# tech-srl/code2vec

Hardware: NVIDIA H100
Metric: path-contexts/sec (train step, batch 1024x200) (higher is better)
Workload: dtype tf32 operands / fp32 accumulate+storage

## Files before the change

### code2vec_b200/csrc/engine.cu

```cuda
#include <cuda_runtime.h>
#include <math.h>
#include <stdio.h>
#include <stdlib.h>
#include <string.h>

#include <string>
#include <utility>
#include <vector>

#include "../../include/c2v_b200.h"
#include "common.cuh"
#include "kernels.cuh"
#include "sgemm.cuh"
#include "umma_gemm.cuh"

using namespace c2v;

namespace {

thread_local std::string g_create_error = "";

constexpr size_t kAlign = 256;
inline size_t align_up(size_t x, size_t a = kAlign) { return (x + a - 1) / a * a; }

// ... 875 lines not shown
    C2V_CUDA(e, cudaEventRecord(e->ev_fork, st));
    C2V_CUDA(e, cudaStreamWaitEvent(e->side, e->ev_fork, 0));
    {
      PhaseTimer pt(e, PH_DX_SCATTER, e->side);
      BucketPlan bp;
      if (e->inbox.world > 1 && plan_buckets(e, &bp, true)) {
        if (e->sorted_src != cs.src || e->sorted_rows != cs.rows) {
          if ((rc = sort_entries(e, e->side, cs, bp))) return rc;
        }
        e->sorted_src = nullptr;
        const int32_t* starts = wsp<int32_t>(e, e->ws.bkt_starts);
        C2V_LAUNCH(e, (inbox_counts_kernel<<<1, 32, 0, e->side>>>(e->inbox, bp, starts)));
        C2V_LAUNCH(e, (scatter_inbox_kernel<<<(3 * N + 7) / 8, 256, 0, e->side>>>(cs, dp, mask, wsp<int32_t>(e, e->ws.perm), starts, bp, dXg,
                                                                              e->inbox, e->grad_scale)));
      } else if (plan_buckets(e, &bp)) {
        if ((rc = sort_entries(e, e->side, cs, bp))) return rc;
        C2V_LAUNCH(e, (scatter_sorted_kernel<<<(3 * N + 7) / 8, 256, 0, e->side>>>(cs, dp, mask, wsp<int32_t>(e, e->ws.perm), dXg, e->gr_tok,
                                                                               e->gr_path, e->grad_scale)));
      } else if (e->deterministic) {
        if ((rc = det_scatter(e, e->side, cs, mask, dp, dXg, false))) return rc;
      } else {
        C2V_LAUNCH(e, (scatter_dx_kernel<<<(N + 7) / 8, 256, 0, e->side>>>(cs, dp, mask, dXg, e->gr_tok, e->gr_path, e->grad_scale)));
      }
    }
    if ((rc = early_catchup(e, e->side))) return rc;
    C2V_CUDA(e, cudaEventRecord(e->ev_join, e->side));
    if ((rc = run_pending_dy(e, st))) return rc;
    {
      PhaseTimer pt(e, PH_DW, st);
      umma::Operand opA{Xg, (size_t)K3, true, x3 ? wsp<float>(e, e->ws.Xg_lo) : nullptr};
      umma::Operand opB{H, (size_t)D, true, H_lo};
      const int ks = umma::effective_splits(N, kSplitDw);
      umma::EpiStore ep{part, (size_t)D, (size_t)K3 * D};
      C2V_LAUNCH(e, C2V_CUDA(e, (umma::launch(st, K3, D, N, kSplitDw, opA, opB, ep, e->num_sms))));
      rc = launch_colsum(e, st, part, (size_t)K3 * D, ks, K3 * D, e->grad.W);
      if (rc) return rc;
    }
    C2V_CUDA(e, cudaStreamWaitEvent(st, e->ev_join, 0));
    if (e->dy_in_flight) {
      C2V_CUDA(e, cudaStreamWaitEvent(st, e->ev_join2, 0));
      e->dy_in_flight = false;
    }
    e->emb_grads_clean = false;
    return C2V_OK;
  }
  {
    PhaseTimer pt(e, PH_DW, st);
    simt::GatherColsX al{cs, dp};
    simt::ColsX bl{H, (size_t)D};
    const int ks = simt::effective_ksplit(N, kSplitDw);
    simt::StoreC ep{part, (size_t)D, (size_t)K3 * D};
    C2V_LAUNCH(e, C2V_CUDA(e, simt::launch(st, K3, D, N, kSplitDw, al, bl, ep)));
    rc = launch_colsum(e, st, part, (size_t)K3 * D, ks, K3 * D, e->grad.W);
    if (rc) return rc;
  }
  {
    if (e->lazy) {
      if (e->lazy_grads_pending)
        return fail(e, C2V_ERR_STATE, "lazy_adam: every train step must be followed by c2v_adam_step before the next one");
      e->lazy_grads_pending = true;
    } else if (!e->emb_grads_clean && e->table_world == 1) {
      C2V_CUDA(e, cudaMemsetAsync(e->grad.tok, 0, (size_t)e->dims.token_vocab * d * 4, st));
      C2V_CUDA(e, cudaMemsetAsync(e->grad.path, 0, (size_t)e->dims.path_vocab * d * 4, st));
    }
    PhaseTimer pt(e, PH_DX_SCATTER, st);
    simt::RowsK al{H, (size_t)D};
    simt::RowsK bl{e->theta.W, (size_t)D};
// ... 40 lines not shown
  }
  simt::RowsK al{S, e->ws.ldS};
  simt::ColsX bl{e->theta.tgt, (size_t)D};
  const int ks = simt::effective_ksplit(Y, kSplitDv);
  simt::StoreC ep{part, (size_t)D, (size_t)B * D};
  C2V_LAUNCH(e, C2V_CUDA(e, simt::launch(st, B, D, Y, kSplitDv, al, bl, ep)));
  return launch_colsum(e, st, part, (size_t)B * D, ks, B * D, dv);
}

int run_dy(c2v_engine* e, cudaStream_t st, const float* v, int B, const SlabDesc& slab) {
  const int D = e->dims.code_dim, Y = e->dims.target_vocab;
  float* S = wsp<float>(e, e->ws.S);
  {
    PhaseTimer pt(e, PH_DY, st);
    if (is_3x(e) && !aligned16(v))
      return fail(e, C2V_ERR_INVALID, "3xTF32: the code vectors must be 16-byte aligned");
    if (is_tc(e) && aligned16(v)) {
      const size_t ldB = align_up((size_t)B, 4);
      int rcs;
      if (is_3x(e)) {
        PhaseTimer pts(e, PH_SPLIT, st);
        rcs = transpose_operand(e, st, v, B, D, ldB, e->ws.vT, true, e->ws.vT_lo);
      } else {
        rcs = transpose_operand(e, st, v, B, D, ldB, e->ws.vT, false);
      }
      if (rcs) return rcs;
      umma::Operand opA{S, e->ws.ldS, true, is_3x(e) ? wsp<float>(e, e->ws.S_lo) : nullptr};
      umma::Operand opB{wsp<float>(e, e->ws.vT), ldB, false, is_3x(e) ? wsp<float>(e, e->ws.vT_lo) : nullptr};
      auto go = [&](auto ep) -> int {
        if (slab.loaders)
          C2V_LAUNCH(e, C2V_CUDA(e, (umma::launch_cfg<true, false, decltype(ep), umma::AXSoftmaxGrad<false>>(
                                        st, Y, D, B, 1, opA, opB, ep, e->num_sms, umma::AXSoftmaxGrad<false>{slab.sg}))));
        else
          C2V_LAUNCH(e, C2V_CUDA(e, (umma::launch_cfg<true, false, decltype(ep)>(st, Y, D, B, 1, opA, opB, ep, e->num_sms))));
        return C2V_OK;
      };
      int rc;
      if (e->tgt_armed && e->has_adam) {
        const double lr_t = (double)e->tgt_lr * sqrt(1.0 - pow((double)e->tgt_b2, (double)e->tgt_t)) /
                            (1.0 - pow((double)e->tgt_b1, (double)e->tgt_t));
        if ((rc = go(umma::EpiAdam{e->theta.tgt, e->am.tgt, e->av.tgt, (size_t)D, (float)lr_t, e->tgt_b1, e->tgt_b2, e->tgt_eps,
                                   1.f - e->tgt_b1, 1.f - e->tgt_b2, e->adam_epi_prefetch})))
          return rc;
        e->tgt_armed = false;
        e->tgt_fused_t = e->tgt_t;
        e->tgt_t_valid = false;
      } else if ((rc = go(umma::EpiStore{e->grad.tgt, (size_t)D, 0}))) {
        return rc;
      }
    } else {
      simt::ColsX al{S, e->ws.ldS};
      simt::ColsX bl{v, (size_t)D};
      simt::StoreC ep{e->grad.tgt, (size_t)D, 0};
      C2V_LAUNCH(e, C2V_CUDA(e, simt::launch(st, Y, D, B, 1, al, bl, ep)));
    }
  }
  if (e->ev_tgt_ready) C2V_CUDA(e, cudaEventRecord(e->ev_tgt_ready, st));
  return C2V_OK;
}

int target_grad_gemms(c2v_engine* e, cudaStream_t st, const float* v, int B, float* dv, const SlabDesc& slab) {
  int rc = run_dv(e, st, B, dv, slab);
  if (rc) return rc;
  if (e->dy_late == 2 && is_tc(e)) {
    C2V_CUDA(e, cudaEventRecord(e->ev_fork2, st));
    C2V_CUDA(e, cudaStreamWaitEvent(e->side2, e->ev_fork2, 0));
    if ((rc = run_dy(e, e->side2, v, B, slab))) return rc;
// ... 972 lines not shown
  C2V_CUDA(e, cudaMemcpyAsync(pth, h_path, nb, cudaMemcpyHostToDevice, st));
  C2V_CUDA(e, cudaMemcpyAsync(tgt, h_tgt, nb, cudaMemcpyHostToDevice, st));
  C2V_CUDA(e, cudaMemcpyAsync(mask, h_mask, nb, cudaMemcpyHostToDevice, st));
  const Dropout dp = make_dropout(e->dims, 1.0f, 0, 0, nullptr);
  if ((rc = forward_impl(e, st, src, pth, tgt, mask, B, dp, code, attn))) return rc;
  if ((rc = topk_impl(e, st, code, B, tki, tkv, normalize))) return rc;
  const int Y = e->dims.target_vocab;
  const int k = e->dims.top_k < Y ? e->dims.top_k : Y;
  C2V_CUDA(e, cudaMemcpyAsync(h_topk_idx, tki, (size_t)B * k * 4, cudaMemcpyDeviceToHost, st));
  C2V_CUDA(e, cudaMemcpyAsync(h_topk_val, tkv, (size_t)B * k * 4, cudaMemcpyDeviceToHost, st));
  if (h_code_vec) C2V_CUDA(e, cudaMemcpyAsync(h_code_vec, code, (size_t)B * e->dims.code_dim * 4, cudaMemcpyDeviceToHost, st));
  if (h_attn) C2V_CUDA(e, cudaMemcpyAsync(h_attn, attn, nb, cudaMemcpyDeviceToHost, st));
  C2V_CUDA(e, cudaStreamSynchronize(st));
  return C2V_OK;
}

int c2v_selftest_gemm(c2v_engine* e, int32_t a_mn, int32_t b_mn, int32_t bn, int32_t M, int32_t N, int32_t K,
                      int32_t splits, const float* A, size_t lda, const float* Bm, size_t ldb, float* C, size_t ldc,
                      void* stream) {
  return c2v_selftest_gemm3(e, a_mn, b_mn, bn, M, N, K, splits, A, nullptr, lda, Bm, nullptr, ldb, C, ldc, stream);
}

int c2v_selftest_gemm3(c2v_engine* e, int32_t a_mn, int32_t b_mn, int32_t bn, int32_t M, int32_t N, int32_t K,
                       int32_t splits, const float* A, const float* A_lo, size_t lda, const float* Bm, const float* B_lo,
                       size_t ldb, float* C, size_t ldc, void* stream) {
  if (!e || !A || !Bm || !C) return C2V_ERR_INVALID;
  if ((A_lo != nullptr) != (B_lo != nullptr)) return fail(e, C2V_ERR_INVALID, "3xTF32 needs the low parts of both operands");
  C2V_CUDA(e, cudaSetDevice(e->device));
  cudaStream_t st = (cudaStream_t)stream;
  umma::Operand opA{A, lda, a_mn != 0, A_lo};
  umma::Operand opB{Bm, ldb, b_mn != 0, B_lo};
  if (!umma::operand_ok(opA) || !umma::operand_ok(opB)) return fail(e, C2V_ERR_INVALID, "operand not TMA-compatible");
  umma::EpiStore ep{C, ldc, (size_t)M * ldc};
  if (bn != 192 && bn != 256) return fail(e, C2V_ERR_INVALID, "bn must be 192 or 256");
  C2V_LAUNCH(e, C2V_CUDA(e, (umma::launch(st, M, N, K, splits, opA, opB, ep, e->num_sms))));
  return umma::effective_splits(K, splits);
}

int c2v_selftest_split(c2v_engine* e, const float* x, float* hi, float* lo, size_t count, void* stream) {
  if (!e || !x || !hi || !lo) return C2V_ERR_INVALID;
  if (count % 4 || ((uintptr_t)x | (uintptr_t)hi | (uintptr_t)lo) % 16) return fail(e, C2V_ERR_INVALID, "count % 4 and 16-byte alignment");
  C2V_CUDA(e, cudaSetDevice(e->device));
  size_t blocks = (count / 4 + 255) / 256;
  if (blocks > (size_t)e->num_sms * 16) blocks = (size_t)e->num_sms * 16;
  if (blocks < 1) blocks = 1;
  C2V_LAUNCH(e, (split_tf32_kernel<<<(unsigned)blocks, 256, 0, (cudaStream_t)stream>>>(x, hi, lo, count / 4)));
  return C2V_OK;
}

int c2v_selftest_transpose(c2v_engine* e, const float* x, int32_t rows, int32_t cols, float* xT, float* xT_lo, size_t ldT,
                           void* stream) {
  if (!e || !x || !xT) return C2V_ERR_INVALID;
  if (rows < 1 || cols < 1 || ldT < (size_t)rows || cols > 65535 * 32) return fail(e, C2V_ERR_INVALID, "bad size");
  C2V_CUDA(e, cudaSetDevice(e->device));
  const dim3 grid((unsigned)((rows + 31) / 32), (unsigned)((cols + 31) / 32));
  cudaStream_t st = (cudaStream_t)stream;
  if (xT_lo) C2V_LAUNCH(e, (transpose_kernel<true><<<grid, 256, 0, st>>>(x, rows, cols, xT, xT_lo, ldT, nullptr, nullptr)));
  else C2V_LAUNCH(e, (transpose_kernel<false><<<grid, 256, 0, st>>>(x, rows, cols, xT, nullptr, ldT, nullptr, nullptr)));
  return C2V_OK;
}

int c2v_selftest_row_sum(c2v_engine* e, int32_t table_id, const int32_t* rows, const float* vals, int32_t count, float* out,
                         void* stream) {
  if (!e || !rows || !vals || !out) return C2V_ERR_INVALID;
  if (!e->wbase) return fail(e, C2V_ERR_STATE, "workspace not bound (c2v_bind_workspace)");
  if (table_id != 0 && table_id != 1) return fail(e, C2V_ERR_INVALID, "table_id must be 0 (token table) or 1 (path table)");
  if (count < 0 || (int64_t)count > 3ll * e->dims.max_batch * e->dims.max_contexts)
    return fail(e, C2V_ERR_INVALID, "count must be in [0, 3 * max_batch * max_contexts]");
// ... 35 lines not shown
```

### code2vec_b200/csrc/umma_gemm.cuh

```cuda
#pragma once
#include <cuda.h>
#include <cuda_runtime.h>
#include <limits.h>
#include <stdint.h>

#include "common.cuh"

namespace c2v {
namespace umma {

constexpr int BM = 128;
constexpr int BN = 128;
constexpr int BK = 32;
constexpr int WG_K = 8;
constexpr int STAGES = 4;
constexpr int kThreads = 4 * 128;
constexpr int kRegsProducer = 72;
constexpr int kRegsConsumer = 128;
constexpr int kRegsEpilogue = 184;
static_assert(kRegsProducer + 2 * kRegsConsumer + kRegsEpilogue == 4 * 128, "the roles share the CTA's registers");

__device__ __forceinline__ float fast_tanh(float x) {
  float e, r;
  asm("ex2.approx.ftz.f32 %0, %1;" : "=f"(e) : "f"(x * 2.885390081777927f));
  asm("rcp.approx.ftz.f32 %0, %1;" : "=f"(r) : "f"(e + 1.f));
  return fmaf(-2.f, r, 1.f);
}

__device__ __forceinline__ uint32_t smem_u32(const void* p) { return (uint32_t)__cvta_generic_to_shared(p); }

__device__ __forceinline__ void mbar_init(uint64_t* bar, uint32_t count) {
  asm volatile("mbarrier.init.shared::cta.b64 [%0], %1;" ::"r"(smem_u32(bar)), "r"(count));
}
__device__ __forceinline__ void mbar_expect_tx(uint64_t* bar, uint32_t bytes) {
  asm volatile("mbarrier.expect_tx.relaxed.cta.shared::cta.b64 [%0], %1;" ::"r"(smem_u32(bar)), "r"(bytes) : "memory");
}
__device__ __forceinline__ void mbar_arrive(uint64_t* bar) {
  asm volatile("mbarrier.arrive.shared::cta.b64 _, [%0];" ::"r"(smem_u32(bar)) : "memory");
}
__device__ __forceinline__ void mbar_arrive_expect_tx(uint64_t* bar, uint32_t bytes) {
  asm volatile("mbarrier.arrive.expect_tx.shared::cta.b64 _, [%0], %1;" ::"r"(smem_u32(bar)), "r"(bytes) : "memory");
}
__device__ __forceinline__ bool mbar_try_wait(uint64_t* bar, uint32_t parity) {
  uint32_t ok;
  asm volatile(
      "{\n\t.reg .pred p;\n\t"
      "mbarrier.try_wait.parity.shared::cta.b64 p, [%1], %2;\n\t"
      "selp.u32 %0, 1, 0, p;\n\t}"
// ... 20 lines not shown
      "cp.async.bulk.tensor.2d.shared::cluster.global.mbarrier::complete_tx::bytes [%0], [%1, {%3, %4}], [%2];"
      ::"r"(smem_u32(smem_dst)), "l"(map), "r"(smem_u32(bar)), "r"(c0), "r"(c1) : "memory");
}

__device__ __forceinline__ uint64_t gmma_desc(uint32_t saddr) {
  return (uint64_t)((saddr >> 4) & 0x3FFF) | (1ull << 16) | ((uint64_t)(1024 >> 4) << 32) | (1ull << 62);
}
__device__ __forceinline__ void wg_fence() { asm volatile("wgmma.fence.sync.aligned;" ::: "memory"); }
__device__ __forceinline__ void wg_commit() { asm volatile("wgmma.commit_group.sync.aligned;" ::: "memory"); }
template <int N>
__device__ __forceinline__ void wg_wait() { asm volatile("wgmma.wait_group.sync.aligned %0;" ::"n"(N) : "memory"); }
template <int R>
__device__ __forceinline__ void wg_regs_dec() { asm volatile("setmaxnreg.dec.sync.aligned.u32 %0;" ::"n"(R)); }
template <int R>
__device__ __forceinline__ void wg_regs_inc() { asm volatile("setmaxnreg.inc.sync.aligned.u32 %0;" ::"n"(R)); }
__device__ __forceinline__ void wgmma_tf32(float (&d)[64], uint64_t da, uint64_t db, uint32_t accumulate) {
  asm volatile(
      "{\n\t.reg .pred p;\n\t"
      "setp.ne.b32 p, %66, 0;\n\t"
      "wgmma.mma_async.sync.aligned.m64n128k8.f32.tf32.tf32 "
      "{%0, %1, %2, %3, %4, %5, %6, %7, %8, %9, %10, %11, %12, %13, %14, %15, %16, %17, %18, %19, %20, %21, %22, %23, "
      "%24, %25, %26, %27, %28, %29, %30, %31, %32, %33, %34, %35, %36, %37, %38, %39, %40, %41, %42, %43, %44, %45, "
      "%46, %47, %48, %49, %50, %51, %52, %53, %54, %55, %56, %57, %58, %59, %60, %61, %62, %63}, %64, %65, p, 1, 1;\n\t}"
      : "+f"(d[0]), "+f"(d[1]), "+f"(d[2]), "+f"(d[3]), "+f"(d[4]), "+f"(d[5]), "+f"(d[6]), "+f"(d[7]), "+f"(d[8]),
        "+f"(d[9]), "+f"(d[10]), "+f"(d[11]), "+f"(d[12]), "+f"(d[13]), "+f"(d[14]), "+f"(d[15]), "+f"(d[16]),
        "+f"(d[17]), "+f"(d[18]), "+f"(d[19]), "+f"(d[20]), "+f"(d[21]), "+f"(d[22]), "+f"(d[23]), "+f"(d[24]),
        "+f"(d[25]), "+f"(d[26]), "+f"(d[27]), "+f"(d[28]), "+f"(d[29]), "+f"(d[30]), "+f"(d[31]), "+f"(d[32]),
        "+f"(d[33]), "+f"(d[34]), "+f"(d[35]), "+f"(d[36]), "+f"(d[37]), "+f"(d[38]), "+f"(d[39]), "+f"(d[40]),
        "+f"(d[41]), "+f"(d[42]), "+f"(d[43]), "+f"(d[44]), "+f"(d[45]), "+f"(d[46]), "+f"(d[47]), "+f"(d[48]),
        "+f"(d[49]), "+f"(d[50]), "+f"(d[51]), "+f"(d[52]), "+f"(d[53]), "+f"(d[54]), "+f"(d[55]), "+f"(d[56]),
        "+f"(d[57]), "+f"(d[58]), "+f"(d[59]), "+f"(d[60]), "+f"(d[61]), "+f"(d[62]), "+f"(d[63])
      : "l"(da), "l"(db), "r"(accumulate));
}

struct EpiNoState {};

struct EpiStore {
  using State = EpiNoState;
  float* C;
  size_t ldc;
  size_t split_stride;
  __device__ __forceinline__ void begin(State&) const {}
  __device__ __forceinline__ void end(int, int, int, bool, State&) const {}
  __device__ __forceinline__ void observe(int, int, const uint32_t (&)[32], int, State&) const {}
  __device__ __forceinline__ float map(float x) const { return x; }
  __device__ __forceinline__ float* out(int split) const { return C + (size_t)split * split_stride; }
  using Pre = EpiNoState;
  static constexpr int kRowBatch = 8;
  static constexpr bool kMoveRegs = false;
  __device__ __forceinline__ void prefetch(const float*, size_t, Pre&) const {}
  __device__ __forceinline__ void store4(float* c, size_t off, float4 v, const Pre&) const { *reinterpret_cast<float4*>(c + off) = v; }
  __device__ __forceinline__ void store1(float* c, size_t off, float x) const { c[off] = x; }
};
template <bool PRECISE>
struct EpiTanhStoreT {
  using State = EpiNoState;
  float* C;
  size_t ldc;
  __device__ __forceinline__ void begin(State&) const {}
  __device__ __forceinline__ void end(int, int, int, bool, State&) const {}
  __device__ __forceinline__ void observe(int, int, const uint32_t (&)[32], int, State&) const {}
  __device__ __forceinline__ float map(float x) const { return PRECISE ? tanhf(x) : fast_tanh(x); }
  __device__ __forceinline__ float* out(int) const { return C; }
  using Pre = EpiNoState;
  static constexpr int kRowBatch = 8;
  __device__ __forceinline__ void prefetch(const float*, size_t, Pre&) const {}
// ... 474 lines not shown
  const int32_t* ids = seg == 0 ? g.cs.src : seg == 1 ? g.cs.pth : g.cs.tgt;
  const int K = 3 * g.cs.d;
  float4 v[8];
#pragma unroll
  for (int i = 0; i < 8; ++i) {
    const int m = m0 + rg + 16 * i;
    v[i] = make_float4(0.f, 0.f, 0.f, 0.f);
    if (m < M) v[i] = ld4(((seg == 1) ? table_row(g.cs.path, ids[m], g.cs.d) : table_row(g.cs.tok, ids[m], g.cs.d)) + col);
  }
#pragma unroll
  for (int i = 0; i < 8; ++i) {
    const int r = rg + 16 * i, m = m0 + r;
    if (g.dp.enabled) {
      const float4 mlt = dropout_mult4(g.dp, m, kb * (BK / 4) + c);
      v[i].x *= mlt.x; v[i].y *= mlt.y; v[i].z *= mlt.z; v[i].w *= mlt.w;
    }
    *reinterpret_cast<float4*>(dst + r * 128 + ((c ^ (r & 7)) << 4)) = v[i];
    if (write_x && m < M) *reinterpret_cast<float4*>(g.Xout + (size_t)m * K + kb * BK + c * 4) = v[i];
  }
}

struct GemmShape {
  int M, N, K;
  int m_tiles, n_tiles, splits;
  int kblocks_per_split;
  int n_fastest;
  int terms;
};
struct GemmPtrs {
  const float* a;
  size_t lda;
};

struct SmemLayout {
  static constexpr int kABytes = BM * BK * 4;
  static constexpr int kBBytes = BN * BK * 4;
  static constexpr int kStageBytes = kABytes + kBBytes;
  static constexpr int kEpiOffset = STAGES * kStageBytes;
  static constexpr int kEpiBytes = 64 * BN * 4;
  static constexpr int kBarOffset = kEpiOffset + 2 * kEpiBytes;
  static constexpr int kTotal = kBarOffset + 256 + 1024;
  static_assert((3 * STAGES + 2) * 8 <= 256, "the barriers fit their block");
  static_assert(kTotal <= 232448, "exceeds the 227 KB of shared memory a CTA can opt into");
};

template <bool A_MN, bool B_MN, class Epi, class AX = AXNone>
__global__ void __launch_bounds__(kThreads, 1)
umma_gemm_kernel(const __grid_constant__ CUtensorMap tmA, const __grid_constant__ CUtensorMap tmB,
                 const __grid_constant__ CUtensorMap tmAlo, const __grid_constant__ CUtensorMap tmBlo, GemmShape gs,
                 GemmPtrs ptr, Epi epi, AX ax = AX{}) {
  if (epi_gate_closed(epi, 0)) return;
  using L = SmemLayout;
  static_assert(!(A_MN && AX::kKind == 2), "the gathered A tile is K-major");
  constexpr bool kTmaA = !A_MN && AX::kKind == 0;
  constexpr bool kTmaB = !B_MN;
  constexpr uint32_t kTxBytes = (kTmaA ? L::kABytes : 0) + (kTmaB ? L::kBBytes : 0);
  constexpr uint32_t kMnTxBytes = (A_MN ? L::kABytes : 0) + (B_MN ? L::kBBytes : 0);
  constexpr int kLag = kMnTxBytes ? STAGES - 2 : 0;
  static_assert(kLag <= STAGES - 2, "the producer would wait for a stage only a step it has not published can free");
  extern __shared__ uint8_t smem_raw[];
  uint8_t* smem = reinterpret_cast<uint8_t*>((reinterpret_cast<uintptr_t>(smem_raw) + 1023) & ~(uintptr_t)1023);
  uint64_t* full_bar = reinterpret_cast<uint64_t*>(smem + L::kBarOffset);
  uint64_t* empty_bar = full_bar + STAGES;
  uint64_t* landed_bar = empty_bar + STAGES;
  uint64_t* epi_full = landed_bar + STAGES;
  uint64_t* epi_empty = epi_full + 1;

  const int wg = threadIdx.x >> 7, warp = threadIdx.x >> 5, lane = threadIdx.x & 31;
  const int total_items = gs.m_tiles * gs.n_tiles * gs.splits;
  const int total_kblocks = (gs.K + BK - 1) / BK;

  if (threadIdx.x == 0) {
    for (int s = 0; s < STAGES; ++s) { mbar_init(&full_bar[s], 128); mbar_init(&empty_bar[s], 8); mbar_init(&landed_bar[s], 1); }
    mbar_init(epi_full, 256);
    mbar_init(epi_empty, 128);
    asm volatile("fence.mbarrier_init.release.cluster;" ::: "memory");
  }
  __syncthreads();

  auto decode = [&](int item, int& mt, int& nt, int& sp) {
    if (gs.n_fastest) {
      nt = item % gs.n_tiles;
      const int r = item / gs.n_tiles;
      mt = r % gs.m_tiles;
      sp = r / gs.m_tiles;
// ... 10 lines not shown
    const int t = threadIdx.x;
    struct Cursor {
      int item, mt, nt, kb, kb0, kb1, pass;
      int stage;
      uint32_t phase;
    };
    auto seek = [&](Cursor& c) {
      for (; c.item < total_items; c.item += gridDim.x) {
        int sp;
        decode(c.item, c.mt, c.nt, sp);
        c.kb = c.kb0 = sp * gs.kblocks_per_split;
        c.kb1 = min(total_kblocks, c.kb0 + gs.kblocks_per_split);
        c.pass = gs.terms == 3 ? 0 : 2;
        if (c.kb0 < c.kb1) return;
      }
    };
    auto next = [&](Cursor& c) {
      if (++c.stage == STAGES) { c.stage = 0; c.phase ^= 1; }
      if (++c.kb < c.kb1) return;
      if (c.pass < 2) { ++c.pass; c.kb = c.kb0; return; }
      c.item += gridDim.x;
      seek(c);
    };
    auto issue = [&](const Cursor& c) {
      mbar_wait(&empty_bar[c.stage], c.phase ^ 1);
      uint8_t* sa = smem + c.stage * L::kStageBytes;
      uint8_t* sb = sa + L::kABytes;
      const int k0 = c.kb * BK;
      const bool a_lo = c.pass == 0, b_lo = c.pass == 1;
      if (t == 0) {
        if (kTxBytes) {
          mbar_expect_tx(&full_bar[c.stage], kTxBytes);
          if (kTmaA) tma_load_2d(sa, a_lo ? &tmAlo : &tmA, &full_bar[c.stage], k0, c.mt * BM);
          if (kTmaB) tma_load_2d(sb, b_lo ? &tmBlo : &tmB, &full_bar[c.stage], k0, c.nt * BN);
        }
        if (kMnTxBytes) {
          mbar_arrive_expect_tx(&landed_bar[c.stage], kMnTxBytes);
#pragma unroll
          for (int q = 0; q < 4; ++q) {
            if (A_MN) tma_load_2d(sa + q * 4096, a_lo ? &tmAlo : &tmA, &landed_bar[c.stage], c.mt * BM + 32 * q, k0);
            if (B_MN) tma_load_2d(sb + q * 4096, b_lo ? &tmBlo : &tmB, &landed_bar[c.stage], c.nt * BN + 32 * q, k0);
          }
        }
      }
      if constexpr (AX::kKind == 2) load_tile_gather(sa, ax, c.mt * BM, gs.M, c.kb, ax.Xout != nullptr && c.nt == 0, t);
      else if constexpr (!A_MN && !kTmaA) load_tile_k(sa, ptr.a, ptr.lda, c.mt * BM, gs.M, k0, gs.K, t, ax);
    };
    auto complete = [&](const Cursor& c) {
      uint8_t* sa = smem + c.stage * L::kStageBytes;
      uint8_t* sb = sa + L::kABytes;
      if constexpr (kMnTxBytes != 0) {
        if constexpr (A_MN && AX::kKind == 1) {
          const int k0 = c.kb * BK, x = c.mt * BM + 32 * warp + lane;
          float ce = 0.f;
          int te = -1;
          if (k0 + lane < gs.K) ax.example(k0 + lane, ce, te);
          mbar_wait(&landed_bar[c.stage], c.phase);
          transpose_box(sa + warp * 4096, lane, [&](float s, int k) {
            const float ck = __shfl_sync(0xffffffffu, ce, k);
            const int tk = __shfl_sync(0xffffffffu, te, k);
            return (x < gs.M && k0 + k < gs.K) ? ax.p(s, x, ck, tk) : 0.f;
          });
        } else {
          mbar_wait(&landed_bar[c.stage], c.phase);
          if constexpr (A_MN) transpose_box(sa + warp * 4096, lane, [](float s, int) { return s; });
        }
        if constexpr (B_MN) transpose_box(sb + warp * 4096, lane, [](float s, int) { return s; });
      }
      if constexpr (!kTmaA || !kTmaB) fence_proxy_async_smem();
      mbar_arrive(&full_bar[c.stage]);
    };
    Cursor ld{static_cast<int>(blockIdx.x), 0, 0, 0, 0, 0, 0, 0, 0u};
    seek(ld);
    if constexpr (kLag == 0) {
      for (; ld.item < total_items; next(ld)) { issue(ld); complete(ld); }
    } else {
      Cursor tr = ld;
      for (int ahead = 0; tr.item < total_items;) {
        const bool more = ld.item < total_items;
        if (more) { issue(ld); next(ld); ++ahead; }
        if (ahead > kLag || !more) { complete(tr); next(tr); --ahead; }
      }
    }
  } else if (wg <= 2) {
    const int cw = wg - 1, wl = warp & 3;
    const int g = lane >> 2;
    const uint32_t stg_row = smem_u32(smem + L::kEpiOffset + cw * L::kEpiBytes) + (wl >> 1) * 4096 + (16 * (wl & 1) + g) * 128 +
                             ((g ^ ((lane >> 1) & 1)) << 4) + 8 * (lane & 1);
    int stage = 0;
    uint32_t phase = 0, epi_phase = 0;
    float acc[64];
    for (int item = blockIdx.x; item < total_items; item += gridDim.x, epi_phase ^= 1) {
      int mt, nt, sp;
      decode(item, mt, nt, sp);
      const int kb0 = sp * gs.kblocks_per_split;
      const int kb1 = min(total_kblocks, kb0 + gs.kblocks_per_split);
      const int n_steps = (kb1 - kb0) * gs.terms;
      int prev = 0;
      for (int it = 0; it < n_steps; ++it) {
        mbar_wait(&full_bar[stage], phase);
        const uint32_t sa = smem_u32(smem + stage * L::kStageBytes) + cw * 64 * 128;
        const uint32_t sb = smem_u32(smem + stage * L::kStageBytes + L::kABytes);
        wg_fence();
#pragma unroll
        for (int k = 0; k < BK / WG_K; ++k)
          wgmma_tf32(acc, gmma_desc(sa + k * WG_K * 4), gmma_desc(sb + k * WG_K * 4), (it > 0 || k > 0) ? 1u : 0u);
        wg_commit();
        wg_wait<1>();
        if (it > 0 && lane == 0) mbar_arrive(&empty_bar[prev]);
        prev = stage;
        if (++stage == STAGES) { stage = 0; phase ^= 1; }
      }
      wg_wait<0>();
      if (n_steps > 0 && lane == 0) mbar_arrive(&empty_bar[prev]);

      mbar_wait(epi_empty, epi_phase ^ 1);
#pragma unroll
      for (int j = 0; j < BN / 8; ++j) {
#pragma unroll
        for (int i = 0; i < 2; ++i)
          asm volatile("st.shared.v2.f32 [%0], {%1, %2};" ::"r"((stg_row ^ ((j & 3) << 5)) + 8192 * (j >> 2) + 1024 * i),
                       "f"(acc[4 * j + 2 * i]), "f"(acc[4 * j + 2 * i + 1]) : "memory");
      }
      mbar_arrive(epi_full);
    }
  } else {
    if constexpr (epi_move_regs<Epi>(0)) wg_regs_inc<kRegsEpilogue>();
    const int w = warp & 3;
    float* stg = reinterpret_cast<float*>(smem + L::kEpiOffset + (w >> 1) * L::kEpiBytes);
    auto prefetch_item = [&](int it) {
      if (it >= total_items) return;
      int mt2, nt2, sp2;
      decode(it, mt2, nt2, sp2);
      epi_prefetch_tile(epi, mt2 * BM + 32 * w + lane, nt2 * BN, BN, gs.M, gs.N, 0);
    };
    prefetch_item(blockIdx.x);
    uint32_t epi_phase = 0;
    for (int item = blockIdx.x; item < total_items; item += gridDim.x, epi_phase ^= 1) {
      int mt, nt, sp;
      decode(item, mt, nt, sp);
      prefetch_item(item + gridDim.x);
      mbar_wait<true>(epi_full, epi_phase);
      const int m_base = mt * BM + 32 * w, m = m_base + lane;
      float* cbase = epi.out(sp);
#pragma unroll 1
      for (int p = 0; p < 2; ++p) {
        typename Epi::State est;
        epi.begin(est);
#pragma unroll 1
        for (int q = p; q < 4; q += 2) {
          float* blk = stg + ((w & 1) | (q << 1)) * 1024;
          uint32_t r[32];
#pragma unroll
          for (int c4 = 0; c4 < 8; ++c4) {
            const float4 x = *reinterpret_cast<const float4*>(blk + lane * 32 + ((c4 ^ (lane & 7)) << 2));
            r[4 * c4] = __float_as_uint(x.x); r[4 * c4 + 1] = __float_as_uint(x.y);
            r[4 * c4 + 2] = __float_as_uint(x.z); r[4 * c4 + 3] = __float_as_uint(x.w);
          }
          __syncwarp();
          const int n = nt * BN + 32 * q;
          if (n < gs.N) {
            if (m < gs.M) epi.observe(m, n, r, gs.N - n, est);
            if (epi_stores<Epi>(0)) store_chunk(epi, est, r, blk, lane, m_base, n, gs.M, gs.N, cbase, epi.ldc);
          }
        }
        epi.end(m, 2 * nt + p, sp, m < gs.M, est);
      }
      mbar_arrive(epi_empty);
    }
  }
}

typedef CUresult (*EncodeTiledFn)(CUtensorMap*, CUtensorMapDataType, cuuint32_t, void*, const cuuint64_t*, const cuuint64_t*,
                                  const cuuint32_t*, const cuuint32_t*, CUtensorMapInterleave, CUtensorMapSwizzle,
                                  CUtensorMapL2promotion, CUtensorMapFloatOOBfill);

inline EncodeTiledFn get_encode_fn() {
  static EncodeTiledFn fn = nullptr;
  if (!fn) {
    void* p = nullptr;
    cudaDriverEntryPointQueryResult qres;
    if (cudaGetDriverEntryPoint("cuTensorMapEncodeTiled", &p, cudaEnableDefault, &qres) == cudaSuccess && p)
      fn = reinterpret_cast<EncodeTiledFn>(p);
  }
  return fn;
}

struct TensorMapKey {
  const float* base;
  uint64_t rows, cols, ld;
  uint32_t box_rows;
  bool operator==(const TensorMapKey& o) const {
    return base == o.base && rows == o.rows && cols == o.cols && ld == o.ld && box_rows == o.box_rows;
// ... 3 lines not shown
  static constexpr int kCap = 96;
  TensorMapKey key[kCap];
  CUtensorMap map[kCap];
  int n = 0, next = 0;
};
inline bool make_tensor_map(CUtensorMap* map, const float* base, uint64_t rows, uint64_t cols, uint64_t ld, uint32_t box_rows) {
  static thread_local TensorMapCache cache;
  const TensorMapKey k{base, rows, cols, ld, box_rows};
  for (int i = 0; i < cache.n; ++i)
    if (cache.key[i] == k) { *map = cache.map[i]; return true; }
  EncodeTiledFn fn = get_encode_fn();
  if (!fn) return false;
  cuuint64_t dims[2] = {cols, rows};
  cuuint64_t strides[1] = {ld * sizeof(float)};
  cuuint32_t box[2] = {32, box_rows};
  cuuint32_t estr[2] = {1, 1};
  CUresult r = fn(map, CU_TENSOR_MAP_DATA_TYPE_FLOAT32, 2, const_cast<float*>(base), dims, strides, box, estr,
                  CU_TENSOR_MAP_INTERLEAVE_NONE, CU_TENSOR_MAP_SWIZZLE_128B, CU_TENSOR_MAP_L2_PROMOTION_L2_256B,
                  CU_TENSOR_MAP_FLOAT_OOB_FILL_NONE);
  if (r != CUDA_SUCCESS) return false;
  const int slot = (cache.n < TensorMapCache::kCap) ? cache.n++ : (cache.next++ % TensorMapCache::kCap);
  cache.key[slot] = k;
  cache.map[slot] = *map;
  return true;
}

struct Operand {
  const float* base;
  size_t ld;
  bool major_mn;
  const float* lo = nullptr;
};

inline bool operand_map(CUtensorMap* map, const float* base, bool major_mn, int X, int K, size_t ld) {
  return major_mn ? make_tensor_map(map, base, (uint64_t)K, (uint64_t)X, ld, BK) : make_tensor_map(map, base, (uint64_t)X, (uint64_t)K, ld, BM);
}

inline GemmShape make_shape(int M, int N, int K, int splits, int terms) {
  GemmShape gs;
  gs.M = M; gs.N = N; gs.K = K;
  gs.terms = terms;
  gs.m_tiles = (M + BM - 1) / BM;
  gs.n_tiles = (N + BN - 1) / BN;
  const int total_kblocks = (K + BK - 1) / BK;
  if (splits < 1) splits = 1;
  if (splits > total_kblocks) splits = total_kblocks;
  gs.kblocks_per_split = (total_kblocks + splits - 1) / splits;
  gs.splits = (total_kblocks + gs.kblocks_per_split - 1) / gs.kblocks_per_split;
  gs.n_fastest = (gs.n_tiles < gs.m_tiles) ? 1 : 0;
  return gs;
}

template <bool A_MN, bool B_MN, class Epi, class AX>
inline cudaError_t launch_kernel(cudaStream_t st, const CUtensorMap& tmA, const CUtensorMap& tmB, const CUtensorMap& tmAlo,
                                 const CUtensorMap& tmBlo, const GemmShape& gs, const GemmPtrs& ptr, const Epi& epi, int num_sms,
                                 const AX& ax) {
  auto kern = umma_gemm_kernel<A_MN, B_MN, Epi, AX>;
  cudaError_t e = cudaFuncSetAttribute(kern, cudaFuncAttributeMaxDynamicSharedMemorySize, SmemLayout::kTotal);
  if (e != cudaSuccess) return e;
  int grid = gs.m_tiles * gs.n_tiles * gs.splits;
  if (grid > num_sms) grid = num_sms;
  kern<<<grid, kThreads, SmemLayout::kTotal, st>>>(tmA, tmB, tmAlo, tmBlo, gs, ptr, epi, ax);
  return cudaGetLastError();
}

template <bool A_MN, bool B_MN, class Epi, class AX = AXNone>
inline cudaError_t launch_cfg(cudaStream_t st, int M, int N, int K, int splits, const Operand& A, const Operand& B, const Epi& epi,
                              int num_sms, const AX& ax = AX{}) {
  CUtensorMap tmA{}, tmB{}, tmAlo{}, tmBlo{};
  const bool three = A.lo != nullptr && B.lo != nullptr;
  if ((A.lo != nullptr) != (B.lo != nullptr)) return cudaErrorInvalidValue;
  if (AX::kKind != 0 && three) return cudaErrorInvalidValue;
  if (A_MN || AX::kKind == 0) {
    if (!operand_map(&tmA, A.base, A_MN, M, K, A.ld)) return cudaErrorInvalidValue;
    if (three && !operand_map(&tmAlo, A.lo, A_MN, M, K, A.ld)) return cudaErrorInvalidValue;
  }
  if (!operand_map(&tmB, B.base, B_MN, N, K, B.ld)) return cudaErrorInvalidValue;
  if (three && !operand_map(&tmBlo, B.lo, B_MN, N, K, B.ld)) return cudaErrorInvalidValue;
  const GemmPtrs ptr{A.base, A.ld};
  return launch_kernel<A_MN, B_MN, Epi, AX>(st, tmA, tmB, tmAlo, tmBlo, make_shape(M, N, K, splits, three ? 3 : 1), ptr, epi,
                                            num_sms, ax);
}

inline int effective_splits(int K, int splits) {
  const int total_kblocks = (K + BK - 1) / BK;
  if (splits < 1) splits = 1;
  if (splits > total_kblocks) splits = total_kblocks;
  const int per = (total_kblocks + splits - 1) / splits;
  return (total_kblocks + per - 1) / per;
}

inline int lse_slots(int n) { return 2 * ((n + BN - 1) / BN); }

template <class Epi>
inline cudaError_t launch(cudaStream_t st, int M, int N, int K, int splits, const Operand& A, const Operand& B, const Epi& epi,
                          int num_sms) {
  if (!A.major_mn && !B.major_mn) return launch_cfg<false, false, Epi>(st, M, N, K, splits, A, B, epi, num_sms);
  if (!A.major_mn && B.major_mn) return launch_cfg<false, true, Epi>(st, M, N, K, splits, A, B, epi, num_sms);
  if (A.major_mn && !B.major_mn) return launch_cfg<true, false, Epi>(st, M, N, K, splits, A, B, epi, num_sms);
  return launch_cfg<true, true, Epi>(st, M, N, K, splits, A, B, epi, num_sms);
}

template <class Epi>
inline cudaError_t launch_ctx_fused(cudaStream_t st, int M, int N, const float* W, size_t ldw, const ContextSource& cs,
                                    const Dropout& dp, float* Xout, const Epi& epi, int num_sms) {
  const int K = 3 * cs.d;
  GemmShape gs = make_shape(M, N, K, 1, 1);
  gs.n_fastest = 1;
  const CUtensorMap none{};
  CUtensorMap tmW{};
  if (!operand_map(&tmW, W, true, N, K, ldw)) return cudaErrorInvalidValue;
  return launch_kernel<false, true, Epi, AXGather>(st, none, tmW, none, none, gs, GemmPtrs{nullptr, 0}, epi, num_sms, AXGather{cs, dp, Xout});
}

inline bool operand_ok(const Operand& o) {
  return (reinterpret_cast<uintptr_t>(o.base) % 16 == 0) && (o.ld % 4 == 0);
}

}
}
```

Baseline: 31.27 million.

## Add 192-column wide GEMM tile variant for dW and target-gradient GEMMs

Templates the warp-specialized wgmma GEMM on tile width and adds a 192-column variant using m64n192k8 instructions, with 3 pipeline stages to fit shared memory. The dW GEMM and the plain target-gradient GEMM now launch with the wide tile. The wider tile raises reuse of A per load and cuts the number of N tiles, for example covering D=384 in two tiles. In exchange it uses more accumulator registers, has a shallower pipeline, and gives fewer work items for the split or persistent schedule.

```diff
diff --git a/code2vec_b200/csrc/engine.cu b/code2vec_b200/csrc/engine.cu
--- a/code2vec_b200/csrc/engine.cu
+++ b/code2vec_b200/csrc/engine.cu
@@ -931,7 +931,8 @@
       umma::Operand opB{H, (size_t)D, true, H_lo};
       const int ks = umma::effective_splits(N, kSplitDw);
       umma::EpiStore ep{part, (size_t)D, (size_t)K3 * D};
-      C2V_LAUNCH(e, C2V_CUDA(e, (umma::launch(st, K3, D, N, kSplitDw, opA, opB, ep, e->num_sms))));
+      C2V_LAUNCH(e, C2V_CUDA(e, (umma::launch_cfg<true, true, umma::EpiStore, umma::AXNone, umma::BN_WIDE>(st, K3, D, N, kSplitDw, opA, opB, ep,
+                                                                                                          e->num_sms))));
       rc = launch_colsum(e, st, part, (size_t)K3 * D, ks, K3 * D, e->grad.W);
       if (rc) return rc;
     }
@@ -1038,7 +1039,8 @@
           C2V_LAUNCH(e, C2V_CUDA(e, (umma::launch_cfg<true, false, decltype(ep), umma::AXSoftmaxGrad<false>>(
                                         st, Y, D, B, 1, opA, opB, ep, e->num_sms, umma::AXSoftmaxGrad<false>{slab.sg}))));
         else
-          C2V_LAUNCH(e, C2V_CUDA(e, (umma::launch_cfg<true, false, decltype(ep)>(st, Y, D, B, 1, opA, opB, ep, e->num_sms))));
+          C2V_LAUNCH(e, C2V_CUDA(e, (umma::launch_cfg<true, false, decltype(ep), umma::AXNone, umma::BN_WIDE>(st, Y, D, B, 1, opA, opB, ep,
+                                                                                                              e->num_sms))));
         return C2V_OK;
       };
       int rc;
@@ -2077,8 +2079,12 @@
   umma::Operand opB{Bm, ldb, b_mn != 0, B_lo};
   if (!umma::operand_ok(opA) || !umma::operand_ok(opB)) return fail(e, C2V_ERR_INVALID, "operand not TMA-compatible");
   umma::EpiStore ep{C, ldc, (size_t)M * ldc};
-  if (bn != 192 && bn != 256) return fail(e, C2V_ERR_INVALID, "bn must be 192 or 256");
-  C2V_LAUNCH(e, C2V_CUDA(e, (umma::launch(st, M, N, K, splits, opA, opB, ep, e->num_sms))));
+  if (bn != 128 && bn != 192 && bn != 256) return fail(e, C2V_ERR_INVALID, "bn must be 128, 192 or 256");
+  if (bn == umma::BN_WIDE) {
+    C2V_LAUNCH(e, C2V_CUDA(e, (umma::launch<umma::EpiStore, umma::BN_WIDE>(st, M, N, K, splits, opA, opB, ep, e->num_sms))));
+  } else {
+    C2V_LAUNCH(e, C2V_CUDA(e, (umma::launch(st, M, N, K, splits, opA, opB, ep, e->num_sms))));
+  }
   return umma::effective_splits(K, splits);
 }
 
diff --git a/code2vec_b200/csrc/umma_gemm.cuh b/code2vec_b200/csrc/umma_gemm.cuh
--- a/code2vec_b200/csrc/umma_gemm.cuh
+++ b/code2vec_b200/csrc/umma_gemm.cuh
@@ -4,6 +4,8 @@
 #include <limits.h>
 #include <stdint.h>
 
+#include <type_traits>
+
 #include "common.cuh"
 
 namespace c2v {
@@ -11,9 +13,9 @@
 
 constexpr int BM = 128;
 constexpr int BN = 128;
+constexpr int BN_WIDE = 192;
 constexpr int BK = 32;
 constexpr int WG_K = 8;
-constexpr int STAGES = 4;
 constexpr int kThreads = 4 * 128;
 constexpr int kRegsProducer = 72;
 constexpr int kRegsConsumer = 128;
@@ -100,6 +102,30 @@
         "+f"(d[57]), "+f"(d[58]), "+f"(d[59]), "+f"(d[60]), "+f"(d[61]), "+f"(d[62]), "+f"(d[63])
       : "l"(da), "l"(db), "r"(accumulate));
 }
+__device__ __forceinline__ void wgmma_tf32(float (&d)[96], uint64_t da, uint64_t db, uint32_t accumulate) {
+  asm volatile(
+      "{\n\t.reg .pred p;\n\t"
+      "setp.ne.b32 p, %98, 0;\n\t"
+      "wgmma.mma_async.sync.aligned.m64n192k8.f32.tf32.tf32 "
+      "{%0, %1, %2, %3, %4, %5, %6, %7, %8, %9, %10, %11, %12, %13, %14, %15, %16, %17, %18, %19, %20, %21, %22, %23, "
+      "%24, %25, %26, %27, %28, %29, %30, %31, %32, %33, %34, %35, %36, %37, %38, %39, %40, %41, %42, %43, %44, %45, "
+      "%46, %47, %48, %49, %50, %51, %52, %53, %54, %55, %56, %57, %58, %59, %60, %61, %62, %63, %64, %65, %66, %67, "
+      "%68, %69, %70, %71, %72, %73, %74, %75, %76, %77, %78, %79, %80, %81, %82, %83, %84, %85, %86, %87, %88, %89, "
+      "%90, %91, %92, %93, %94, %95}, %96, %97, p, 1, 1;\n\t}"
+      : "+f"(d[0]), "+f"(d[1]), "+f"(d[2]), "+f"(d[3]), "+f"(d[4]), "+f"(d[5]), "+f"(d[6]), "+f"(d[7]), "+f"(d[8]),
+        "+f"(d[9]), "+f"(d[10]), "+f"(d[11]), "+f"(d[12]), "+f"(d[13]), "+f"(d[14]), "+f"(d[15]), "+f"(d[16]),
+        "+f"(d[17]), "+f"(d[18]), "+f"(d[19]), "+f"(d[20]), "+f"(d[21]), "+f"(d[22]), "+f"(d[23]), "+f"(d[24]),
+        "+f"(d[25]), "+f"(d[26]), "+f"(d[27]), "+f"(d[28]), "+f"(d[29]), "+f"(d[30]), "+f"(d[31]), "+f"(d[32]),
+        "+f"(d[33]), "+f"(d[34]), "+f"(d[35]), "+f"(d[36]), "+f"(d[37]), "+f"(d[38]), "+f"(d[39]), "+f"(d[40]),
+        "+f"(d[41]), "+f"(d[42]), "+f"(d[43]), "+f"(d[44]), "+f"(d[45]), "+f"(d[46]), "+f"(d[47]), "+f"(d[48]),
+        "+f"(d[49]), "+f"(d[50]), "+f"(d[51]), "+f"(d[52]), "+f"(d[53]), "+f"(d[54]), "+f"(d[55]), "+f"(d[56]),
+        "+f"(d[57]), "+f"(d[58]), "+f"(d[59]), "+f"(d[60]), "+f"(d[61]), "+f"(d[62]), "+f"(d[63]), "+f"(d[64]),
+        "+f"(d[65]), "+f"(d[66]), "+f"(d[67]), "+f"(d[68]), "+f"(d[69]), "+f"(d[70]), "+f"(d[71]), "+f"(d[72]),
+        "+f"(d[73]), "+f"(d[74]), "+f"(d[75]), "+f"(d[76]), "+f"(d[77]), "+f"(d[78]), "+f"(d[79]), "+f"(d[80]),
+        "+f"(d[81]), "+f"(d[82]), "+f"(d[83]), "+f"(d[84]), "+f"(d[85]), "+f"(d[86]), "+f"(d[87]), "+f"(d[88]),
+        "+f"(d[89]), "+f"(d[90]), "+f"(d[91]), "+f"(d[92]), "+f"(d[93]), "+f"(d[94]), "+f"(d[95])
+      : "l"(da), "l"(db), "r"(accumulate));
+}
 
 struct EpiNoState {};
 
@@ -640,25 +666,32 @@
   size_t lda;
 };
 
+template <int TN>
 struct SmemLayout {
+  static constexpr int kStages = TN == BN ? 4 : 3;
   static constexpr int kABytes = BM * BK * 4;
-  static constexpr int kBBytes = BN * BK * 4;
+  static constexpr int kBBytes = TN * BK * 4;
   static constexpr int kStageBytes = kABytes + kBBytes;
-  static constexpr int kEpiOffset = STAGES * kStageBytes;
-  static constexpr int kEpiBytes = 64 * BN * 4;
+  static constexpr int kEpiOffset = kStages * kStageBytes;
+  static constexpr int kEpiBytes = 64 * TN * 4;
   static constexpr int kBarOffset = kEpiOffset + 2 * kEpiBytes;
   static constexpr int kTotal = kBarOffset + 256 + 1024;
-  static_assert((3 * STAGES + 2) * 8 <= 256, "the barriers fit their block");
+  static_assert(TN == BN || TN == BN_WIDE, "the tile is 128 or 192 columns wide");
+  static_assert(kStageBytes % 1024 == 0 && kEpiBytes % 4096 == 0, "the swizzled tiles and staging blocks stay 1024-byte aligned");
+  static_assert((3 * kStages + 2) * 8 <= 256, "the barriers fit their block");
   static_assert(kTotal <= 232448, "exceeds the 227 KB of shared memory a CTA can opt into");
 };
 
-template <bool A_MN, bool B_MN, class Epi, class AX = AXNone>
+template <bool A_MN, bool B_MN, class Epi, class AX = AXNone, int TN = BN>
 __global__ void __launch_bounds__(kThreads, 1)
 umma_gemm_kernel(const __grid_constant__ CUtensorMap tmA, const __grid_constant__ CUtensorMap tmB,
                  const __grid_constant__ CUtensorMap tmAlo, const __grid_constant__ CUtensorMap tmBlo, GemmShape gs,
                  GemmPtrs ptr, Epi epi, AX ax = AX{}) {
   if (epi_gate_closed(epi, 0)) return;
-  using L = SmemLayout;
+  using L = SmemLayout<TN>;
+  constexpr int STAGES = L::kStages;
+  static_assert(TN == BN || (std::is_same<typename Epi::State, EpiNoState>::value && AX::kKind == 0),
+                "the wide tile takes neither row-wise epilogue state nor a computed A operand");
   static_assert(!(A_MN && AX::kKind == 2), "the gathered A tile is K-major");
   constexpr bool kTmaA = !A_MN && AX::kKind == 0;
   constexpr bool kTmaB = !B_MN;
@@ -735,14 +768,14 @@
         if (kTxBytes) {
           mbar_expect_tx(&full_bar[c.stage], kTxBytes);
           if (kTmaA) tma_load_2d(sa, a_lo ? &tmAlo : &tmA, &full_bar[c.stage], k0, c.mt * BM);
-          if (kTmaB) tma_load_2d(sb, b_lo ? &tmBlo : &tmB, &full_bar[c.stage], k0, c.nt * BN);
+          if (kTmaB) tma_load_2d(sb, b_lo ? &tmBlo : &tmB, &full_bar[c.stage], k0, c.nt * TN);
         }
         if (kMnTxBytes) {
           mbar_arrive_expect_tx(&landed_bar[c.stage], kMnTxBytes);
 #pragma unroll
-          for (int q = 0; q < 4; ++q) {
-            if (A_MN) tma_load_2d(sa + q * 4096, a_lo ? &tmAlo : &tmA, &landed_bar[c.stage], c.mt * BM + 32 * q, k0);
-            if (B_MN) tma_load_2d(sb + q * 4096, b_lo ? &tmBlo : &tmB, &landed_bar[c.stage], c.nt * BN + 32 * q, k0);
+          for (int q = 0; q < TN / 32; ++q) {
+            if (A_MN && q < BM / 32) tma_load_2d(sa + q * 4096, a_lo ? &tmAlo : &tmA, &landed_bar[c.stage], c.mt * BM + 32 * q, k0);
+            if (B_MN) tma_load_2d(sb + q * 4096, b_lo ? &tmBlo : &tmB, &landed_bar[c.stage], c.nt * TN + 32 * q, k0);
           }
         }
       }
@@ -768,7 +801,12 @@
           mbar_wait(&landed_bar[c.stage], c.phase);
           if constexpr (A_MN) transpose_box(sa + warp * 4096, lane, [](float s, int) { return s; });
         }
-        if constexpr (B_MN) transpose_box(sb + warp * 4096, lane, [](float s, int) { return s; });
+        if constexpr (B_MN) {
+          transpose_box(sb + warp * 4096, lane, [](float s, int) { return s; });
+          if constexpr (TN > BN) {
+            if (warp < TN / 32 - 4) transpose_box(sb + (warp + 4) * 4096, lane, [](float s, int) { return s; });
+          }
+        }
       }
       if constexpr (!kTmaA || !kTmaB) fence_proxy_async_smem();
       mbar_arrive(&full_bar[c.stage]);
@@ -792,7 +830,7 @@
                              ((g ^ ((lane >> 1) & 1)) << 4) + 8 * (lane & 1);
     int stage = 0;
     uint32_t phase = 0, epi_phase = 0;
-    float acc[64];
+    float acc[TN / 2];
     for (int item = blockIdx.x; item < total_items; item += gridDim.x, epi_phase ^= 1) {
       int mt, nt, sp;
       decode(item, mt, nt, sp);
@@ -819,7 +857,7 @@
 
       mbar_wait(epi_empty, epi_phase ^ 1);
 #pragma unroll
-      for (int j = 0; j < BN / 8; ++j) {
+      for (int j = 0; j < TN / 8; ++j) {
 #pragma unroll
         for (int i = 0; i < 2; ++i)
           asm volatile("st.shared.v2.f32 [%0], {%1, %2};" ::"r"((stg_row ^ ((j & 3) << 5)) + 8192 * (j >> 2) + 1024 * i),
@@ -835,7 +873,7 @@
       if (it >= total_items) return;
       int mt2, nt2, sp2;
       decode(it, mt2, nt2, sp2);
-      epi_prefetch_tile(epi, mt2 * BM + 32 * w + lane, nt2 * BN, BN, gs.M, gs.N, 0);
+      epi_prefetch_tile(epi, mt2 * BM + 32 * w + lane, nt2 * TN, TN, gs.M, gs.N, 0);
     };
     prefetch_item(blockIdx.x);
     uint32_t epi_phase = 0;
@@ -851,7 +889,7 @@
         typename Epi::State est;
         epi.begin(est);
 #pragma unroll 1
-        for (int q = p; q < 4; q += 2) {
+        for (int q = p; q < TN / 32; q += 2) {
           float* blk = stg + ((w & 1) | (q << 1)) * 1024;
           uint32_t r[32];
 #pragma unroll
@@ -861,7 +899,7 @@
             r[4 * c4 + 2] = __float_as_uint(x.z); r[4 * c4 + 3] = __float_as_uint(x.w);
           }
           __syncwarp();
-          const int n = nt * BN + 32 * q;
+          const int n = nt * TN + 32 * q;
           if (n < gs.N) {
             if (m < gs.M) epi.observe(m, n, r, gs.N - n, est);
             if (epi_stores<Epi>(0)) store_chunk(epi, est, r, blk, lane, m_base, n, gs.M, gs.N, cbase, epi.ldc);
@@ -931,16 +969,17 @@
   const float* lo = nullptr;
 };
 
-inline bool operand_map(CUtensorMap* map, const float* base, bool major_mn, int X, int K, size_t ld) {
-  return major_mn ? make_tensor_map(map, base, (uint64_t)K, (uint64_t)X, ld, BK) : make_tensor_map(map, base, (uint64_t)X, (uint64_t)K, ld, BM);
-}
-
-inline GemmShape make_shape(int M, int N, int K, int splits, int terms) {
+inline bool operand_map(CUtensorMap* map, const float* base, bool major_mn, int X, int K, size_t ld, int rows = BM) {
+  return major_mn ? make_tensor_map(map, base, (uint64_t)K, (uint64_t)X, ld, BK)
+                  : make_tensor_map(map, base, (uint64_t)X, (uint64_t)K, ld, (uint32_t)rows);
+}
+
+inline GemmShape make_shape(int M, int N, int K, int splits, int terms, int tn = BN) {
   GemmShape gs;
   gs.M = M; gs.N = N; gs.K = K;
   gs.terms = terms;
   gs.m_tiles = (M + BM - 1) / BM;
-  gs.n_tiles = (N + BN - 1) / BN;
+  gs.n_tiles = (N + tn - 1) / tn;
   const int total_kblocks = (K + BK - 1) / BK;
   if (splits < 1) splits = 1;
   if (splits > total_kblocks) splits = total_kblocks;
@@ -950,20 +989,21 @@
   return gs;
 }
 
-template <bool A_MN, bool B_MN, class Epi, class AX>
+template <bool A_MN, bool B_MN, class Epi, class AX, int TN = BN>
 inline cudaError_t launch_kernel(cudaStream_t st, const CUtensorMap& tmA, const CUtensorMap& tmB, const CUtensorMap& tmAlo,
                                  const CUtensorMap& tmBlo, const GemmShape& gs, const GemmPtrs& ptr, const Epi& epi, int num_sms,
                                  const AX& ax) {
-  auto kern = umma_gemm_kernel<A_MN, B_MN, Epi, AX>;
-  cudaError_t e = cudaFuncSetAttribute(kern, cudaFuncAttributeMaxDynamicSharedMemorySize, SmemLayout::kTotal);
+  auto kern = umma_gemm_kernel<A_MN, B_MN, Epi, AX, TN>;
+  constexpr int smem = SmemLayout<TN>::kTotal;
+  cudaError_t e = cudaFuncSetAttribute(kern, cudaFuncAttributeMaxDynamicSharedMemorySize, smem);
   if (e != cudaSuccess) return e;
   int grid = gs.m_tiles * gs.n_tiles * gs.splits;
   if (grid > num_sms) grid = num_sms;
-  kern<<<grid, kThreads, SmemLayout::kTotal, st>>>(tmA, tmB, tmAlo, tmBlo, gs, ptr, epi, ax);
+  kern<<<grid, kThreads, smem, st>>>(tmA, tmB, tmAlo, tmBlo, gs, ptr, epi, ax);
   return cudaGetLastError();
 }
 
-template <bool A_MN, bool B_MN, class Epi, class AX = AXNone>
+template <bool A_MN, bool B_MN, class Epi, class AX = AXNone, int TN = BN>
 inline cudaError_t launch_cfg(cudaStream_t st, int M, int N, int K, int splits, const Operand& A, const Operand& B, const Epi& epi,
                               int num_sms, const AX& ax = AX{}) {
   CUtensorMap tmA{}, tmB{}, tmAlo{}, tmBlo{};
@@ -974,11 +1014,11 @@
     if (!operand_map(&tmA, A.base, A_MN, M, K, A.ld)) return cudaErrorInvalidValue;
     if (three && !operand_map(&tmAlo, A.lo, A_MN, M, K, A.ld)) return cudaErrorInvalidValue;
   }
-  if (!operand_map(&tmB, B.base, B_MN, N, K, B.ld)) return cudaErrorInvalidValue;
-  if (three && !operand_map(&tmBlo, B.lo, B_MN, N, K, B.ld)) return cudaErrorInvalidValue;
+  if (!operand_map(&tmB, B.base, B_MN, N, K, B.ld, TN)) return cudaErrorInvalidValue;
+  if (three && !operand_map(&tmBlo, B.lo, B_MN, N, K, B.ld, TN)) return cudaErrorInvalidValue;
   const GemmPtrs ptr{A.base, A.ld};
-  return launch_kernel<A_MN, B_MN, Epi, AX>(st, tmA, tmB, tmAlo, tmBlo, make_shape(M, N, K, splits, three ? 3 : 1), ptr, epi,
-                                            num_sms, ax);
+  return launch_kernel<A_MN, B_MN, Epi, AX, TN>(st, tmA, tmB, tmAlo, tmBlo, make_shape(M, N, K, splits, three ? 3 : 1, TN), ptr, epi,
+                                                num_sms, ax);
 }
 
 inline int effective_splits(int K, int splits) {
@@ -991,13 +1031,13 @@
 
 inline int lse_slots(int n) { return 2 * ((n + BN - 1) / BN); }
 
-template <class Epi>
+template <class Epi, int TN = BN>
 inline cudaError_t launch(cudaStream_t st, int M, int N, int K, int splits, const Operand& A, const Operand& B, const Epi& epi,
                           int num_sms) {
-  if (!A.major_mn && !B.major_mn) return launch_cfg<false, false, Epi>(st, M, N, K, splits, A, B, epi, num_sms);
-  if (!A.major_mn && B.major_mn) return launch_cfg<false, true, Epi>(st, M, N, K, splits, A, B, epi, num_sms);
-  if (A.major_mn && !B.major_mn) return launch_cfg<true, false, Epi>(st, M, N, K, splits, A, B, epi, num_sms);
-  return launch_cfg<true, true, Epi>(st, M, N, K, splits, A, B, epi, num_sms);
+  if (!A.major_mn && !B.major_mn) return launch_cfg<false, false, Epi, AXNone, TN>(st, M, N, K, splits, A, B, epi, num_sms);
+  if (!A.major_mn && B.major_mn) return launch_cfg<false, true, Epi, AXNone, TN>(st, M, N, K, splits, A, B, epi, num_sms);
+  if (A.major_mn && !B.major_mn) return launch_cfg<true, false, Epi, AXNone, TN>(st, M, N, K, splits, A, B, epi, num_sms);
+  return launch_cfg<true, true, Epi, AXNone, TN>(st, M, N, K, splits, A, B, epi, num_sms);
 }
 
 template <class Epi>
```

After: 31.59 million, median of 6. 1.0% higher.
